# stella-cv/stella_vslam

Measured on AMD Instinct MI355X. Metric: frames/s ORB-extract+match @640x480,2k kpts, higher is better.
Workload: dtype u8

## Files before the change

stella_vslam_amd/csrc/match_kernels.hip:

```cpp
#include "svgpu_internal.h"
#include <algorithm>
#include <cstdlib>
#include "match_kernels.h"
#include "sv_sort.h"
#include "match_device.h"

namespace {
using namespace svmd;

__global__ void k_hamming_pairs(const uint32_t* __restrict__ a, const uint32_t* __restrict__ b, int n, uint32_t* __restrict__ out) {
    const int i = blockIdx.x * blockDim.x + threadIdx.x;
    if (i >= n) return;
    uint32_t q[8];
#pragma unroll
    for (int k = 0; k < 8; ++k) q[k] = a[(size_t)i * 8 + k];
    out[i] = hamming256(q, b + (size_t)i * 8);
}

__global__ __launch_bounds__(256) void k_hamming_matrix(const uint32_t* __restrict__ d1, int n1, const uint32_t* __restrict__ d2,
                                                        int n2, uint16_t* __restrict__ out) {
    __shared__ uint32_t s_t[256 * 8];
    const int j = blockIdx.x * 256 + threadIdx.x;
    uint32_t q[8] = {0, 0, 0, 0, 0, 0, 0, 0};
    if (j < n2)
// ... 251 lines not shown
    uint32_t wq[4][MF_WQ];
#ifdef SV_MF_PAD
    uint32_t pad[SV_MF_PAD];
#endif
};
__device__ __forceinline__ uint32_t mf_row16_max(uint32_t v) {
    v = max(v, (uint32_t)__builtin_amdgcn_update_dpp(0, (int)v, 0x128, 0xF, 0xF, false));
    v = max(v, (uint32_t)__builtin_amdgcn_update_dpp(0, (int)v, 0x124, 0xF, 0xF, false));
    v = max(v, (uint32_t)__builtin_amdgcn_update_dpp(0, (int)v, 0x122, 0xF, 0xF, false));
    v = max(v, (uint32_t)__builtin_amdgcn_update_dpp(0, (int)v, 0x121, 0xF, 0xF, false));
    return v;
}
__device__ __forceinline__ void mf_drain(MfShared& S, const uint32_t* __restrict__ D2, int q_first, int n2c, int wave, int lane, int n, bool ori) {
    for (int e0 = 0; e0 < n; e0 += 64) {
        const int e = e0 + lane;
        bool live = e < n;
        uint32_t key = 0;
        int ql = 0, slot = 0;
        if (live) {
            const uint32_t ent = S.wq[wave][e];
            const int row = (int)(ent >> 16), col = (int)(ent & 0xFFFFu);
            ql = row + wave * MF_QW;
            const uint32_t* q = D2 + (size_t)min(q_first + row, n2c - 1) * 8;
            const uint4 q0 = *reinterpret_cast<const uint4*>(q), q1 = *reinterpret_cast<const uint4*>(q + 4);
            const uint32_t dist = __popc(q0.x ^ S.raw[0][col]) + __popc(q0.y ^ S.raw[1][col]) + __popc(q0.z ^ S.raw[2][col]) + __popc(q0.w ^ S.raw[3][col])
                                  + __popc(q1.x ^ S.raw[4][col]) + __popc(q1.y ^ S.raw[5][col]) + __popc(q1.z ^ S.raw[6][col]) + __popc(q1.w ^ S.raw[7][col]);
            key = (dist << 16) | (uint32_t)S.ridx[col];
            live = S.live[ql] != 0;
            if (ori) live = live && !(fabsf(angle_diff(S.rang[col], S.qa[ql])) > 30.0f);
            if (live) slot = atomicAdd(&S.cnt[ql], 1);
            if (live && slot < MF_SLOTS) S.list[ql][slot] = key;
        }
        unsigned long long ov = __ballot(live && slot >= MF_SLOTS && key < S.rowmax[ql]);
        while (ov) {
            const int src = __ffsll((long long)ov) - 1;
            ov &= ov - 1;
            const uint32_t k = (uint32_t)__builtin_amdgcn_readlane((int)key, src);
            const int row = __builtin_amdgcn_readlane(ql, src);
            uint32_t* R = S.list[row];
            if (k >= S.rowmax[row]) continue;
            const uint32_t v = lane < MF_SLOTS ? R[lane] : 0u;
            const uint32_t vmax = (uint32_t)__builtin_amdgcn_readfirstlane((int)mf_row16_max(v));
            const int arg = __ffsll((long long)__ballot(lane < MF_SLOTS && v == vmax)) - 1;
            uint32_t w = lane == arg ? min(k, vmax) : v;
            if (k < vmax && lane == 0) R[arg] = k;
            w = mf_row16_max(w);
            if (lane == 0) S.rowmax[row] = w;
        }
    }
}
__global__ __launch_bounds__(256, 3) void k_bf_mfma(BfProblem P) {
    __shared__ __attribute__((aligned(16))) MfShared S;
    const int pair = blockIdx.y;
    const int n1 = P.n1_dev ? P.n1_dev[bf_row1(P, pair) * P.n_stride] : P.n1;
    const int n2 = P.n2_dev ? P.n2_dev[pair * P.n_stride] : P.n2;
    const int n1c = min(n1, P.cap1), n2c = min(n2, P.cap2);
    const int tid = threadIdx.x, lane = tid & 63, wave = tid >> 6;
    const int qb = blockIdx.x * MF_QB, q0 = qb + wave * MF_QW;
    if (qb >= n2c) return;
    const uint32_t* __restrict__ D1 = P.sd1 + (size_t)bf_srow1(P, pair) * P.cap1 * 8;
    const float* __restrict__ A1 = P.sa1 + (size_t)bf_srow1(P, pair) * P.cap1;
    const int* __restrict__ I1 = P.si1 + (size_t)bf_srow1(P, pair) * P.cap1;
    const uint32_t* __restrict__ D2 = P.sd2 + (size_t)pair * P.cap2 * 8;
    const float* __restrict__ A2 = P.sa2 + (size_t)pair * P.cap2;
    const int* __restrict__ I2 = P.si2 + (size_t)pair * P.cap2;
    const int* __restrict__ BS1 = P.bs1 + (size_t)bf_srow1(P, pair) * (BF_BINS + 2);
    const bool ori = P.check_orientation != 0;
    const bool prune = ori && bf_prune1(P, pair) && P.prune_ok[pair * 2 + 1];
    S.cnt[tid] = 0;
    S.rowmax[tid] = 0xFFFFFFFFu;
    int my_j = 0;
    {
        const int q = qb + tid;
        bool live = q < n2c;
        if (live) {
            my_j = I2[q];
            live = !P.valid2 || P.valid2[(size_t)pair * P.cap2 + my_j];
        }
        S.qa[tid] = q < n2c ? A2[q] : 0.f;
        S.live[tid] = live ? 1 : 0;
    }
    const int h = lane >> 5;
    v4i A[2][9];
#pragma unroll
    for (int a = 0; a < 2; ++a) {
        const int q = min(q0 + 32 * a + (lane & 31), n2c - 1);
        int pq = 0;
#pragma unroll
        for (int s = 0; s < 8; ++s) {
            const uint32_t w = D2[(size_t)q * 8 + s];
            pq += __popc(w);
            const uint32_t half = (w >> (16 * h)) & 0xFFFFu;
            A[a][s] = v4i{(int)mf_expand02(half & 15u), (int)mf_expand02((half >> 4) & 15u), (int)mf_expand02((half >> 8) & 15u), (int)mf_expand02(half >> 12)};
        }
        const uint2 pp = mf_pop_pieces(pq, true, min((int)P.dmax, 254));
        A[a][8] = h == 0 ? v4i{(int)pp.x, (int)pp.y, 0, 0} : v4i{0, 0, 0, 0};
    }
    int blo[2], bhi[2], wlo[2], whi[2];
    mf_window(A2, BS1, qb, min(qb + MF_QB, n2c) - 1, n1c, prune, blo, bhi);
    const bool wave_live = q0 < n2c;
    mf_window(A2, BS1, min(q0, n2c - 1), min(q0 + MF_QW, n2c) - 1, n1c, prune, wlo, whi);
    const int lt = tid & 31, lw = tid >> 5;
    auto expand = [&](int buf, int tile, int valid) {
        uint4 lo = {0, 0, 0, 0}, hi = {0, 0, 0, 0};
        if (lt < valid) {
            const uint32_t w = S.raw[lw][tile * MF_TT + lt];
            lo.x = mf_expand01(w & 15u);
            lo.y = mf_expand01((w >> 4) & 15u);
            lo.z = mf_expand01((w >> 8) & 15u);
            lo.w = mf_expand01((w >> 12) & 15u);
            hi.x = mf_expand01((w >> 16) & 15u);
            hi.y = mf_expand01((w >> 20) & 15u);
            hi.z = mf_expand01((w >> 24) & 15u);
            hi.w = mf_expand01(w >> 28);
        }
        uint4* B = reinterpret_cast<uint4*>(S.b[buf]) + lw * 64;
        B[lt] = lo;
        B[32 + lt] = hi;
        if (lw == 0) {
            const uint2 pp = lt < valid ? mf_pop_pieces(S.rpop[tile * MF_TT + lt], false, 0) : make_uint2(0x81010101u, 0x01018181u);
            uint4* B8 = reinterpret_cast<uint4*>(S.b[buf]) + 8 * 64;
            B8[lt] = make_uint4(pp.x, pp.y, 0, 0);
            B8[32 + lt] = make_uint4(0, 0, 0, 0);
        }
    };
    int wq_n = 0;
    unsigned n_mine = 0;
    for (int sg = 0; sg < 2; ++sg) {
        const int lo = blo[sg], hi = bhi[sg];
        for (int cbase = lo; cbase < hi; cbase += MF_CH) {
            const int cn = min(MF_CH, hi - cbase), ntiles = (cn + MF_TT - 1) / MF_TT;
            __syncthreads();
            if (tid < cn) {
                const uint4 d0 = *reinterpret_cast<const uint4*>(D1 + (size_t)(cbase + tid) * 8);
                const uint4 d1 = *reinterpret_cast<const uint4*>(D1 + (size_t)(cbase + tid) * 8 + 4);
                S.rang[tid] = A1[cbase + tid];
                S.ridx[tid] = I1[cbase + tid];
                S.rpop[tid] = __popc(d0.x) + __popc(d0.y) + __popc(d0.z) + __popc(d0.w) + __popc(d1.x) + __popc(d1.y) + __popc(d1.z) + __popc(d1.w);
                S.raw[0][tid] = d0.x;
                S.raw[1][tid] = d0.y;
                S.raw[2][tid] = d0.z;
                S.raw[3][tid] = d0.w;
                S.raw[4][tid] = d1.x;
                S.raw[5][tid] = d1.y;
                S.raw[6][tid] = d1.z;
                S.raw[7][tid] = d1.w;
            }
            __syncthreads();
            expand(0, 0, min(MF_TT, cn));
            __syncthreads();
            for (int t = 0, buf = 0; t < ntiles; ++t, buf ^= 1) {
                const int base = cbase + t * MF_TT, tend = min(base + MF_TT, hi);
                const bool mine = wave_live && ((base < whi[0] && tend > wlo[0]) || (base < whi[1] && tend > wlo[1]));
                if (mine) {
                    const v4i* Bf = reinterpret_cast<const v4i*>(S.b[buf]) + lane;
                    v16i acc0 = {}, acc1 = {};
                    v4i b = Bf[0];
#pragma unroll
                    for (int s = 0; s < 9; ++s) {
                        const v4i bn = Bf[(s < 8 ? s + 1 : 0) * 64];
                        acc0 = __builtin_amdgcn_mfma_i32_32x32x32_i8(A[0][s], b, acc0, 0, 0, 0);
                        acc1 = __builtin_amdgcn_mfma_i32_32x32x32_i8(A[1][s], b, acc1, 0, 0, 0);
                        b = bn;
                    }
                    ++n_mine;
                    if (t + 1 < ntiles) expand(buf ^ 1, t + 1, min(MF_TT, cn - (t + 1) * MF_TT));
                    uint32_t m = 0;
#pragma unroll
                    for (int r = 15; r >= 0; --r) m = __builtin_amdgcn_alignbit(m, (uint32_t)acc1[r], 31);
#pragma unroll
                    for (int r = 15; r >= 0; --r) m = __builtin_amdgcn_alignbit(m, (uint32_t)acc0[r], 31);
                    m = ~m;
                    unsigned long long any = __ballot(m != 0);
                    while (any) {
                        int wq = __builtin_amdgcn_readfirstlane(wq_n);
                        if (wq > MF_WQ - 64) {
                            mf_drain(S, D2, q0, n2c, wave, lane, wq, ori);
                            wq = 0;
                        }
                        if (m) {
                            const uint32_t bit = (uint32_t)__ffs((int)m) - 1u;
                            m &= m - 1u;
                            const uint32_t row = ((bit >> 4) << 5) + (bit & 3u) + ((bit & 12u) << 1) + 4u * (uint32_t)h;
                            const int pq = (int)__builtin_amdgcn_mbcnt_hi((uint32_t)(any >> 32), __builtin_amdgcn_mbcnt_lo((uint32_t)any, 0u));
                            S.wq[wave][wq + pq] = (row << 16) | (uint32_t)(t * MF_TT + (lane & 31));
                        }
                        wq_n = wq + __popcll(any);
                        any = __ballot(m != 0);
                    }
                }
                else if (t + 1 < ntiles) expand(buf ^ 1, t + 1, min(MF_TT, cn - (t + 1) * MF_TT));
                __syncthreads();
            }
            mf_drain(S, D2, q0, n2c, wave, lane, __builtin_amdgcn_readfirstlane(wq_n), ori);
            wq_n = 0;
        }
    }
    if (P.mfma_tiles && lane == 0 && n_mine) atomicAdd(P.mfma_tiles, (unsigned long long)n_mine);
    __syncthreads();
    if (qb + tid < n2c) {
        const int cnt = S.cnt[tid], c = min(cnt, MF_SLOTS);
        uint32_t v[MF_SLOTS];
        const uint4* R = reinterpret_cast<const uint4*>(S.list[tid]);
#pragma unroll
        for (int i = 0; i < MF_SLOTS / 4; ++i) {
            const uint4 x = R[i];
            v[4 * i] = x.x;
            v[4 * i + 1] = x.y;
            v[4 * i + 2] = x.z;
            v[4 * i + 3] = x.w;
        }
#pragma unroll
        for (int i = 0; i < MF_SLOTS; ++i) v[i] = i < c ? v[i] : 0xFFFFFFFFu;
#pragma unroll
        for (int k = 2; k <= MF_SLOTS; k <<= 1)
#pragma unroll
            for (int j = k >> 1; j > 0; j >>= 1)
#pragma unroll
                for (int i = 0; i < MF_SLOTS; ++i) {
                    const int l = i ^ j;
                    if (l > i) {
                        const uint32_t lo = min(v[i], v[l]), hi = max(v[i], v[l]);
                        const bool up = (i & k) == 0;
                        v[i] = up ? lo : hi;
                        v[l] = up ? hi : lo;
                    }
                }
        uint4* G = reinterpret_cast<uint4*>(P.topk + ((size_t)pair * P.cap2 + my_j) * BF_LIST);
#pragma unroll
        for (int i = 0; i < MF_SLOTS / 4; ++i) G[i] = make_uint4(v[4 * i], v[4 * i + 1], v[4 * i + 2], v[4 * i + 3]);
        P.cnt[(size_t)pair * P.cap2 + my_j] = cnt;
    }
}

__device__ int bf_decide(const BfProblem& P, int pair, int j, int n1c, const uint4 head, const uint32_t* tail, int cnt, const int* owner) {
    if (cnt == 0) return -1;
    const int m = min(cnt, P.list_k);
    const bool truncated = cnt > P.list_k;
    auto key_at = [&](int k) -> uint32_t { return k == 0 ? head.x : k == 1 ? head.y : k == 2 ? head.z : k == 3 ? head.w : tail[k - 4]; };
    uint32_t a0 = 0xFFFFFFFFu, a1 = 0xFFFFFFFFu;
    for (int k = 0; k < m; ++k) {
        const uint32_t key = key_at(k);
        if (owner[key & 0xFFFFu] < j) continue;
        if (a0 == 0xFFFFFFFFu) a0 = key;
        else {
            a1 = key;
            break;
        }
    }
    const unsigned d_beyond = truncated ? (key_at(m - 1) >> 16) : P.dmax + 1;
    if (a0 != 0xFFFFFFFFu) {
        const unsigned best = a0 >> 16;
        if (HAMMING_DIST_THR_LOW < best) return -1;
        if (a1 != 0xFFFFFFFFu) return (P.lowe_ratio * (float)(a1 >> 16) < (float)best) ? -1 : (int)(a0 & 0xFFFFu);
        if (P.exhaustive && !truncated) return (P.lowe_ratio * (float)MAX_HAMMING_DIST < (float)best) ? -1 : (int)(a0 & 0xFFFFu);
        if (P.lowe_ratio >= 0.f && !(P.lowe_ratio * (float)d_beyond < (float)best)) return (int)(a0 & 0xFFFFu);
    }
    else {
        if (d_beyond > HAMMING_DIST_THR_LOW) return -1;
    }
    return -3;
}

__device__ int bf_full_row(const BfProblem& P, int pair, int j, int n1c, const int* owner, uint32_t* s_best, uint32_t* s_second) {
    const uint32_t* D1 = P.desc1 + (size_t)bf_row1(P, pair) * P.cap1 * 8;
    const uint32_t* D2 = P.desc2 + ((size_t)pair * P.cap2 + j) * 8;
    uint32_t q[8];
#pragma unroll
    for (int k = 0; k < 8; ++k) q[k] = D2[k];
    const float qa = P.angle2[((size_t)pair * P.cap2 + j) * P.angle_stride];
    if (threadIdx.x == 0) {
        *s_best = 0xFFFFFFFFu;
        *s_second = MAX_HAMMING_DIST;
    }
    __syncthreads();
    uint32_t k1 = 0xFFFFFFFFu;
    unsigned d2 = MAX_HAMMING_DIST;
    for (int i = threadIdx.x; i < n1c; i += blockDim.x) {
        if (owner[i] < j) continue;
        if (P.check_orientation && fabsf(angle_diff(P.angle1[((size_t)bf_row1(P, pair) * P.cap1 + i) * P.angle_stride], qa)) > 30.0f) continue;
        const uint32_t key = (hamming256(q, D1 + (size_t)i * 8) << 16) | (uint32_t)i;
        if (key < k1) {
            d2 = min(d2, k1 >> 16);
            k1 = key;
        }
        else d2 = min(d2, key >> 16);
    }
    if (k1 != 0xFFFFFFFFu) atomicMin(s_best, k1);
    __syncthreads();
    const uint32_t kb = *s_best;
    const unsigned mine = (k1 == kb) ? d2 : min(d2, k1 == 0xFFFFFFFFu ? MAX_HAMMING_DIST : (k1 >> 16));
    if (mine < MAX_HAMMING_DIST) atomicMin(s_second, mine);
    __syncthreads();
    const unsigned second = *s_second;
    __syncthreads();
    if (kb == 0xFFFFFFFFu) return -1;
    const unsigned best = kb >> 16;
    if (HAMMING_DIST_THR_LOW < best) return -1;
    if (P.lowe_ratio * (float)second < (float)best) return -1;
    return (int)(kb & 0xFFFFu);
}

template <int BF_RC, int NT>
__global__ __launch_bounds__(NT) void k_bf_replay(BfProblem P, int* __restrict__ g_owner, int* __restrict__ g_match, int use_lds, int pool_rows) {
    extern __shared__ int s_mem[];
    __shared__ int s_changed, s_nund, s_any_und, s_pool_n;
    __shared__ int s_und[1024];
    __shared__ uint32_t s_best, s_second;
    const int pair = blockIdx.x, tid = threadIdx.x, nthr = blockDim.x;
    const int n1 = P.n1_dev ? P.n1_dev[bf_row1(P, pair) * P.n_stride] : P.n1;
    const int n2 = P.n2_dev ? P.n2_dev[pair * P.n_stride] : P.n2;
    const int n1c = min(n1, P.cap1), n2c = min(n2, P.cap2);
    int* owner = use_lds ? s_mem : g_owner + (size_t)pair * P.cap1;
    int* match = use_lds ? s_mem + P.cap1 : g_match + (size_t)pair * P.cap2;
    uint32_t* pool = reinterpret_cast<uint32_t*>(s_mem + (use_lds ? ((P.cap1 + P.cap2 + 3) & ~3) : 0));
    const uint32_t* T = P.topk + (size_t)pair * P.cap2 * BF_LIST;
    const int* C = P.cnt + (size_t)pair * P.cap2;
    for (int i = tid; i < n1c; i += nthr) owner[i] = 0x7FFFFFFF;
    for (int j = tid; j < n2c; j += nthr) match[j] = -2;
    uint4 head[BF_RC];
    int hcnt[BF_RC];
    const uint32_t* tail[BF_RC];
    if (tid == 0) s_pool_n = 0;
    __syncthreads();
#pragma unroll
    for (int u = 0; u < BF_RC; ++u) {
        const int j = u * nthr + tid;
        hcnt[u] = 0;
        head[u] = make_uint4(0xFFFFFFFFu, 0xFFFFFFFFu, 0xFFFFFFFFu, 0xFFFFFFFFu);
        tail[u] = nullptr;
        if (j < n2c) {
            const uint32_t* R = T + (size_t)j * BF_LIST;
            hcnt[u] = C[j];
            head[u] = *reinterpret_cast<const uint4*>(R);
            tail[u] = R + 4;
        }
    }
#pragma unroll
    for (int u = 0; u < BF_RC; ++u)
        if (hcnt[u] > 4 && pool_rows > 0) {
            const int slot = atomicAdd(&s_pool_n, 1);
            if (slot < pool_rows) {
                const uint32_t* R4 = tail[u];
                uint32_t* D = pool + (size_t)slot * (BF_LIST - 4);
#pragma unroll
                for (int i = 0; i < (BF_LIST - 4) / 4; ++i) reinterpret_cast<uint4*>(D)[i] = reinterpret_cast<const uint4*>(R4)[i];
                tail[u] = D;
            }
        }
    __syncthreads();
    for (int sweep = 0; sweep <= n2c; ++sweep) {
        if (tid == 0) {
            s_changed = 0;
            s_any_und = 0;
            s_nund = 0;
        }
        __syncthreads();
        int dec[BF_RC];
        bool und = false;
#pragma unroll
        for (int u = 0; u < BF_RC; ++u) {
            const int j = u * nthr + tid;
            dec[u] = -1;
            if (j < n2c) {
                dec[u] = bf_decide(P, pair, j, n1c, head[u], tail[u], hcnt[u], owner);
                und = und || dec[u] == -3;
            }
        }
        if (und) s_any_und = 1;
        bool changed = false;
        for (int j = BF_RC * nthr + tid; j < n2c; j += nthr) {
            int d = bf_decide(P, pair, j, n1c, *reinterpret_cast<const uint4*>(T + (size_t)j * BF_LIST), T + (size_t)j * BF_LIST + 4, C[j], owner);
            if (d == -3) {
                s_any_und = 1;
                match[j] = -(match[j] + 10);
            }
            else {
                changed = changed || d != match[j];
                match[j] = d;
            }
        }
        __syncthreads();
        if (s_any_und) {
            for (int j0 = 0; j0 < n2c; j0 += nthr) {
                const int j = j0 + tid, u = j0 / nthr;
                bool need = false;
                if (j < n2c) {
                    if (u < BF_RC) {
                        int du = dec[0];
#pragma unroll
                        for (int v = 1; v < BF_RC; ++v)
                            if (v == u) du = dec[v];
                        need = du == -3;
                    }
                    else need = match[j] <= -8;
                }
                if (need) s_und[atomicAdd(&s_nund, 1)] = j;
                __syncthreads();
                const int nund = s_nund;
                int mine = -3;
                for (int k = 0; k < nund; ++k) {
                    const int ju = s_und[k];
                    const int du = bf_full_row(P, pair, ju, n1c, owner, &s_best, &s_second);
                    if (ju == j) mine = du;
                }
                __syncthreads();
                if (tid == 0) s_nund = 0;
                if (need) {
                    if (u < BF_RC) {
#pragma unroll
                        for (int v = 0; v < BF_RC; ++v)
                            if (v == u) dec[v] = mine;
                    }
                    else {
                        changed = changed || mine != -match[j] - 10;
                        match[j] = mine;
                    }
                }
                __syncthreads();
            }
        }
#pragma unroll
        for (int u = 0; u < BF_RC; ++u) {
            const int j = u * nthr + tid;
            if (j < n2c) {
                changed = changed || dec[u] != match[j];
                match[j] = dec[u];
            }
        }
        if (changed) s_changed = 1;
        __syncthreads();
        if (!s_changed) break;
        for (int i = tid; i < n1c; i += nthr) owner[i] = 0x7FFFFFFF;
        __syncthreads();
        for (int j = tid; j < n2c; j += nthr)
            if (match[j] >= 0) atomicMin(&owner[match[j]], j);
        __syncthreads();
    }
    int32_t* out = P.matched + (size_t)pair * P.cap1;
    for (int i = tid; i < P.cap1; i += nthr) out[i] = -1;
    __syncthreads();
    int local = 0;
    for (int j = tid; j < n2c; j += nthr)
        if (match[j] >= 0) {
            out[match[j]] = j;
            ++local;
        }
    if (tid == 0) s_changed = 0;
    __syncthreads();
    if (local) atomicAdd(&s_changed, local);
    __syncthreads();
    if (tid == 0) P.num[pair] = s_changed;
}

#define CAND_SORT_MAX 1024
__device__ __forceinline__ int cand_total(const CandProblem& P) { return P.cand_total ? *P.cand_total : P.cand_off[P.nq]; }
__device__ __forceinline__ bool cand_sorted(const CandProblem& P, int n) { return n <= CAND_SORT_MAX && P.mode != SVGPU_MATCH_TRIANGULATION && P.mode != SVGPU_MATCH_AREA; }
__global__ void k_cand_dist(CandProblem P) {
    if (P.cap > 0 && cand_total(P) > P.cap) return;
    const int q = blockIdx.x;
    if (P.q_valid && !P.q_valid[q]) return;
    const int lo = P.cand_off[q], hi = P.cand_off[q + 1];
    __shared__ unsigned long long s_key[CAND_SORT_MAX];
    const bool long_sorted = hi - lo > 64 && cand_sorted(P, hi - lo);
    uint32_t qd[8];
#pragma unroll
    for (int k = 0; k < 8; ++k) qd[k] = P.qdesc[(size_t)q * 8 + k];
    for (int c = lo + threadIdx.x; c < hi; c += blockDim.x) {
        const int t = P.cand_idx[c];
        bool gated = (P.cand_skip && P.cand_skip[c]) || (P.occupied && P.occupied[t]);
        if (!gated && P.t_xright && 0.f < P.t_xright[t]) {
            const float err = fabsf(P.q_xright[q] - P.t_xright[t]);
            if (P.q_xr_tol[q] < err) gated = true;
        }
        if (!gated && P.check_orientation && fabsf(angle_diff(P.q_angle[q], P.t_angle[t])) > 30.0f) gated = true;
        if (!gated && P.chi_gate) {
            const double e_x = P.q_reproj[2 * q] - (double)P.t_xy[2 * t], e_y = P.q_reproj[2 * q + 1] - (double)P.t_xy[2 * t + 1];
            const double inv_sigma_sq = (double)P.inv_level_sigma_sq[(unsigned)P.t_octave[t]];
            if (P.chi_t_xright && P.chi_t_xright[t] >= 0.f) {
                const float e_xr = P.q_reproj_xr[q] - P.chi_t_xright[t];
                const double err = (e_x * e_x + e_y * e_y) + (double)(e_xr * e_xr);
                if ((double)7.81473f < err * inv_sigma_sq) gated = true;
            }
            else {
                const double err = e_x * e_x + e_y * e_y;
                if ((double)5.99146f < err * inv_sigma_sq) gated = true;
            }
        }
        uint32_t e = 0xFFFFFFFFu;
        if (!gated) {
            const unsigned d = hamming256(qd, P.tdesc + (size_t)t * 8);
            bool useless = false;
            if (P.mode == SVGPU_MATCH_BEST_ONLY) useless = P.thr < d;
            else if (P.mode == SVGPU_MATCH_RATIO_SAME_OCTAVE) useless = !(P.lowe_ratio * (float)d < (float)P.thr) && P.thr < d;
            e = useless ? 0xFFFFFFFFu : ((uint32_t)d << 22) | (uint32_t)t;
        }
        P.dist[c] = e;
        if (long_sorted) s_key[c - lo] = e == 0xFFFFFFFFu ? ~0ull : ((unsigned long long)(e >> 22) << 32) | ((unsigned long long)(c - lo) << 22) | (e & 0x3FFFFFu);
    }
    const int n = hi - lo;
    if (!cand_sorted(P, n)) return;
    if (n <= 64) {
        const int c = lo + (int)threadIdx.x;
        const uint32_t e = c < hi ? P.dist[c] : 0xFFFFFFFFu;
        unsigned long long key = e == 0xFFFFFFFFu ? ~0ull : ((unsigned long long)(e >> 22) << 32) | ((unsigned long long)threadIdx.x << 22) | (e & 0x3FFFFFu);
        const int lane = threadIdx.x;
#pragma unroll
        for (int k = 2; k <= 64; k <<= 1)
#pragma unroll
            for (int j = k >> 1; j > 0; j >>= 1) {
                const unsigned long long other = __shfl_xor(key, j, 64);
                const bool up = (lane & k) == 0, low = (lane & j) == 0;
                const bool take_min = up == low;
                key = take_min ? (key < other ? key : other) : (key < other ? other : key);
            }
        if (c < hi) P.dist[c] = key == ~0ull ? 0xFFFFFFFFu : ((uint32_t)(key >> 32) << 22) | (uint32_t)(key & 0x3FFFFFu);
        return;
    }
    int npow2 = 128;
    while (npow2 < n) npow2 <<= 1;
    for (int i = n + threadIdx.x; i < npow2; i += 64) s_key[i] = ~0ull;
    __syncthreads();
    for (int k = 2; k <= npow2; k <<= 1)
        for (int j = k >> 1; j > 0; j >>= 1) {
            for (int i = threadIdx.x; i < npow2; i += 64) {
                const int p = i ^ j;
                if (p > i) {
                    const unsigned long long a = s_key[i], b = s_key[p];
                    if ((a > b) == ((i & k) == 0)) {
                        s_key[i] = b;
                        s_key[p] = a;
                    }
                }
            }
            __syncthreads();
        }
    for (int i = threadIdx.x; i < n; i += 64) {
        const unsigned long long key = s_key[i];
        P.dist[lo + i] = key == ~0ull ? 0xFFFFFFFFu : ((uint32_t)(key >> 32) << 22) | (uint32_t)(key & 0x3FFFFFu);
    }
}

__device__ __forceinline__ int cand_verdict(const CandProblem& P, unsigned best, unsigned second, int best_lvl, int second_lvl, int best_idx);
__device__ int cand_decide(const CandProblem& P, int q, const int* owner) {
    if (P.q_valid && !P.q_valid[q]) return -1;
    const int lo = P.cand_off[q], hi = P.cand_cnt ? lo + P.cand_cnt[q] : P.cand_off[q + 1];
    if (lo == hi) return -1;
    const bool tri = P.mode == SVGPU_MATCH_TRIANGULATION;
    unsigned best = tri ? P.thr : MAX_HAMMING_DIST, second = MAX_HAMMING_DIST;
    int best_lvl = -1, second_lvl = -1, best_idx = -1;
    if (cand_sorted(P, hi - lo)) {
        for (int c = lo; c < hi; ++c) {
            const uint32_t e = P.dist[c];
            if (e == 0xFFFFFFFFu) break;
            const unsigned d = e >> 22;
            if (d >= MAX_HAMMING_DIST) break;
            const int t = (int)(e & 0x3FFFFFu);
            if (owner[t] < q) continue;
            if (best_idx < 0) {
                best = d;
                best_idx = t;
                best_lvl = P.t_octave ? P.t_octave[t] : 0;
                if (P.mode == SVGPU_MATCH_BEST_ONLY) break;
            }
            else {
                second = d;
                second_lvl = P.t_octave ? P.t_octave[t] : 0;
                break;
            }
        }
    }
    else {
    auto visit = [&](uint32_t e) {
        if (e == 0xFFFFFFFFu) return;
        const unsigned d = e >> 22;
        const int t = (int)(e & 0x3FFFFFu);
        if (owner[t] < q) return;
        if (tri && (P.thr < d || best < d)) return;
        if (d < best) {
            second = best;
            best = d;
            second_lvl = best_lvl;
            best_lvl = P.t_octave ? P.t_octave[t] : 0;
            best_idx = t;
        }
        else if (d < second) {
            second_lvl = P.t_octave ? P.t_octave[t] : 0;
            second = d;
        }
    };
    for (int c = lo; c < hi; c += 4) {
        const uint32_t e0 = P.dist[c], e1 = c + 1 < hi ? P.dist[c + 1] : 0xFFFFFFFFu, e2 = c + 2 < hi ? P.dist[c + 2] : 0xFFFFFFFFu,
                       e3 = c + 3 < hi ? P.dist[c + 3] : 0xFFFFFFFFu;
        visit(e0);
        visit(e1);
        visit(e2);
        visit(e3);
    }
    }
    return cand_verdict(P, best, second, best_lvl, second_lvl, best_idx);
}

__device__ __forceinline__ int cand_verdict(const CandProblem& P, unsigned best, unsigned second, int best_lvl, int second_lvl, int best_idx) {
    if (P.mode == SVGPU_MATCH_RATIO_SAME_OCTAVE) {
        if (best <= P.thr) {
            if (best_lvl == second_lvl && (float)best > P.lowe_ratio * (float)second) return -1;
            return best_idx;
        }
        return -1;
    }
    if (P.mode == SVGPU_MATCH_BEST_ONLY) {
        if (P.thr < best) return -1;
        return best_idx;
    }
    if (P.thr < best || best_idx < 0) return -1;
    if (P.lowe_ratio * (float)second < (float)best) return -1;
    return best_idx;
}

#define SV_LDS __attribute__((address_space(3)))
struct CandLds {
    SV_LDS int* owner;
    SV_LDS int* match;
    SV_LDS int* off;
    SV_LDS int* cnt;
    SV_LDS uint32_t* head;
    SV_LDS uint8_t* occ;
    SV_LDS uint8_t* lvl;
    SV_LDS uint8_t* qv;
    int K;
};
__device__ __forceinline__ int cand_decide_lds(const CandProblem& P, int q, const CandLds& S) {
    const int lo = S.off[q], n = S.cnt ? S.cnt[q] : S.off[q + 1] - lo;
    if (n == 0 || (S.qv && !S.qv[q])) return -1;
    if (!cand_sorted(P, n)) return cand_decide(P, q, (const int*)S.owner);
    unsigned best = MAX_HAMMING_DIST, second = MAX_HAMMING_DIST;
    int best_lvl = -1, second_lvl = -1, best_idx = -1;
    bool done = false;
    auto take_loaded = [&](uint32_t e, int own, int lv) {
        if (done) return;
        if (e == 0xFFFFFFFFu || (e >> 22) >= MAX_HAMMING_DIST) {
            done = true;
            return;
        }
        const int t = (int)(e & 0x3FFFFFu);
        if (own < q) return;
        if (best_idx < 0) {
            best = e >> 22;
            best_idx = t;
            best_lvl = lv;
            if (P.mode == SVGPU_MATCH_BEST_ONLY) done = true;
        }
        else {
            second = e >> 22;
            second_lvl = lv;
            done = true;
        }
    };
    auto take = [&](uint32_t e) {
        if (done || e == 0xFFFFFFFFu) {
            take_loaded(e, 0, 0);
            return;
        }
        const int t = (int)(e & 0x3FFFFFu);
        take_loaded(e, S.owner[t], S.lvl ? (int)S.lvl[t] : 0);
    };
    const int nk = min(n, S.K);
    const SV_LDS uint32_t* h = S.head + (size_t)q * S.K;
    for (int k0 = 0; k0 < nk && !done; k0 += 4) {
        uint32_t e[4];
        int own[4], lv[4];
#pragma unroll
        for (int j = 0; j < 4; ++j) e[j] = k0 + j < nk ? h[k0 + j] : 0xFFFFFFFFu;
#pragma unroll
        for (int j = 0; j < 4; ++j) {
            const int t = e[j] == 0xFFFFFFFFu ? 0 : (int)(e[j] & 0x3FFFFFu);
            own[j] = S.owner[t];
            lv[j] = S.lvl ? (int)S.lvl[t] : 0;
        }
        const bool best_only = P.mode == SVGPU_MATCH_BEST_ONLY;
#pragma unroll
        for (int j = 0; j < 4; ++j) {
            const unsigned d = e[j] >> 22;
            const bool padding = k0 + j >= nk;
            const bool stop = !padding && (e[j] == 0xFFFFFFFFu || d >= MAX_HAMMING_DIST), active = !done;
            const bool avail = active && !padding && !stop && own[j] >= q, first = avail && best_idx < 0, sec = avail && best_idx >= 0;
            best = first ? d : best;
            best_lvl = first ? lv[j] : best_lvl;
            second = sec ? d : second;
            second_lvl = sec ? lv[j] : second_lvl;
            best_idx = first ? (int)(e[j] & 0x3FFFFFu) : best_idx;
            done = done || (active && stop) || sec || (first && best_only);
        }
    }
    for (int c = lo + nk; c < lo + n && !done; c += 4) {
        const int hi = lo + n;
        const uint32_t e0 = P.dist[c], e1 = c + 1 < hi ? P.dist[c + 1] : 0xFFFFFFFFu, e2 = c + 2 < hi ? P.dist[c + 2] : 0xFFFFFFFFu,
                       e3 = c + 3 < hi ? P.dist[c + 3] : 0xFFFFFFFFu;
        take(e0);
        take(e1);
        take(e2);
        take(e3);
    }
    return cand_verdict(P, best, second, best_lvl, second_lvl, best_idx);
}
#define CAND_LDS_BUDGET (150 * 1024)
__host__ __device__ inline size_t cand_lds_bytes(int nq, int nt, int K, bool with_cnt = false) {
    return (size_t)(nt + nq + nq + 1 + (with_cnt ? nq : 0)) * 4 + (size_t)nq * K * 4 + 2 * (((size_t)nt + 3) & ~size_t(3)) + (((size_t)nq + 3) & ~size_t(3)) + 16;
}
#define CAND_CHUNK_QPT 1
__global__ __launch_bounds__(1024) void k_cand_replay_lds(CandProblem P, int K) {
    extern __shared__ int s_cand[];
    __shared__ int s_changed;
    if (P.cap > 0 && cand_total(P) > P.cap) {
        if (P.num_host && threadIdx.x == 0) P.num_host[0] = 0, P.num_host[1] = cand_total(P);
        return;
    }
    const int tid = threadIdx.x, nthr = blockDim.x;
    const int nt = P.nt_dev ? min(*P.nt_dev, P.nt) : P.nt;
    CandLds S;
    S.owner = (SV_LDS int*)s_cand;
    S.match = S.owner + P.nt;
    S.off = S.match + P.nq;
    S.cnt = P.cand_cnt ? S.off + P.nq + 1 : nullptr;
    S.head = (SV_LDS uint32_t*)(S.off + P.nq + 1 + (P.cand_cnt ? P.nq : 0));
    SV_LDS uint8_t* bytes = (SV_LDS uint8_t*)(S.head + (size_t)P.nq * K);
    S.occ = P.occupied ? bytes : nullptr;
    S.lvl = P.t_octave ? bytes + ((P.nt + 3) & ~3) : nullptr;
    S.qv = P.q_valid ? bytes + 2 * ((P.nt + 3) & ~3) : nullptr;
    S.K = K;
    for (int q = tid; q <= P.nq; q += nthr) {
        S.off[q] = P.cand_off[q];
        if (S.cnt && q < P.nq) S.cnt[q] = P.cand_cnt[q];
        if (S.qv && q < P.nq) S.qv[q] = P.q_valid[q];
    }
    for (int t = tid; t < nt; t += nthr) {
        S.owner[t] = (P.occupied && P.occupied[t]) ? -1 : 0x7FFFFFFF;
        if (S.lvl) S.lvl[t] = (uint8_t)P.t_octave[t];
    }
    S.occ = nullptr;
    __syncthreads();
    for (int i = tid; i < P.nq * K; i += nthr) {
        const int q = i / K, k = i - q * K, lo = S.off[q], n = S.cnt ? S.cnt[q] : S.off[q + 1] - lo;
        if (k < n) S.head[i] = P.dist[lo + k];
    }
    if (tid == 0) s_changed = 0;
    __syncthreads();
    if (P.dbg_phase == 1) return;
    int local = 0, sweeps_total = 0;
    const int chunk = nthr * CAND_CHUNK_QPT;
    for (int lo = 0; lo < P.nq; lo += chunk) {
        int mine[CAND_CHUNK_QPT], prev[CAND_CHUNK_QPT];
#pragma unroll
        for (int u = 0; u < CAND_CHUNK_QPT; ++u) mine[u] = -2, prev[u] = -1;
        for (int sweep = 0; sweep <= chunk; ++sweep) {
// ... 259 lines not shown
        const int t = P.cand_idx[lo + (int)(kb & 0xFFFFFu)];
        if (lane == 0) {
            const int prev = (int)ld(reinterpret_cast<unsigned*>(&holder[t]));
            if (0 <= prev) st(reinterpret_cast<unsigned*>(&match[prev]), 0xFFFFFFFFu);
            st(reinterpret_cast<unsigned*>(&match[q]), (unsigned)t);
            st(reinterpret_cast<unsigned*>(&holder[t]), (unsigned)q);
            st(&mdist[t], best);
        }
        __syncthreads();
    }
    int local = 0;
    __syncthreads();
    for (int q = lane; q < P.nq; q += 64) {
        const int m = (int)ld(reinterpret_cast<const unsigned*>(&match[q]));
        P.match_q[q] = m;
        local += m >= 0;
    }
#pragma unroll
    for (int off = 32; off > 0; off >>= 1) local += __shfl_xor(local, off, 64);
    if (lane == 0) *P.num = local;
}

__device__ __forceinline__ int wave_sum_i(int v) {
#pragma unroll
    for (int off = 32; off > 0; off >>= 1) v += __shfl_xor(v, off, 64);
    return v;
}
struct StereoPair {
    const svgpu_keypoint *kl, *kr;
    const uint32_t *dl, *dr;
    int nl, nr;
    float *xr, *depth, *corr;
    int32_t *row_off, *row_fill, *row_items;
};
__device__ __forceinline__ StereoPair stereo_pair(const StereoProblem& P, int pair) {
    StereoPair Q;
    const size_t o = P.nl_dev ? (size_t)pair * P.cap : 0;
    Q.nl = P.nl_dev ? min(P.nl_dev[(size_t)pair * P.n_stride], P.cap) : P.nl;
    Q.nr = P.nr_dev ? min(P.nr_dev[(size_t)pair * P.n_stride], P.cap) : P.nr;
    Q.kl = P.kl + o, Q.kr = P.kr + o, Q.dl = P.dl + o * 8, Q.dr = P.dr + o * 8;
    Q.xr = P.xr + o, Q.depth = P.depth + o, Q.corr = P.corr + o;
    const int nr_cap = P.nl_dev ? P.cap : P.nr;
    Q.row_off = P.row_off + (size_t)pair * (P.rows + 1);
    Q.row_fill = P.row_fill + (size_t)pair * P.rows;
    Q.row_items = P.row_items + (size_t)pair * nr_cap * P.rows_per_kp;
    return Q;
}
__device__ __forceinline__ void stereo_band(const StereoProblem& P, const svgpu_keypoint& r, int& min_r, int& max_r) {
    const float rad = 2.0f * P.sf[r.octave];
    max_r = min((int)ceil((double)(r.y + rad)), P.rows - 1);
    min_r = max((int)floor((double)(r.y - rad)), 0);
}
template <bool FILL>
__global__ __launch_bounds__(256) void k_stereo_rows(StereoProblem P) {
    const StereoPair Q = stereo_pair(P, blockIdx.y);
    const int ir = blockIdx.x * 256 + threadIdx.x;
    if (ir >= Q.nr) return;
    int min_r, max_r;
    stereo_band(P, Q.kr[ir], min_r, max_r);
    for (int row = min_r; row <= max_r; ++row) {
        if (FILL) Q.row_items[Q.row_off[row] + atomicAdd(&Q.row_fill[row], 1)] = ir;
        else atomicAdd(&Q.row_off[row], 1);
    }
}
__global__ __launch_bounds__(1024) void k_stereo_rows_scan(StereoProblem P) {
    __shared__ int s_part[1024];
    __shared__ int s_carry;
    int32_t* off = P.row_off + (size_t)blockIdx.x * (P.rows + 1);
    const int tid = threadIdx.x, n = P.rows;
    if (tid == 0) s_carry = 0;
    __syncthreads();
    for (int base = 0; base < n; base += 1024) {
        const int i = base + tid;
        const int v = i < n ? off[i] : 0;
        int incl = v;
#pragma unroll
        for (int d = 1; d < 64; d <<= 1) {
            const int t = __shfl_up(incl, d, 64);
            if ((tid & 63) >= d) incl += t;
        }
        if ((tid & 63) == 63) s_part[tid >> 6] = incl;
        __syncthreads();
        int before = 0;
        for (int w = 0; w < (tid >> 6); ++w) before += s_part[w];
        const int carry = s_carry;
        if (i < n) off[i] = carry + before + incl - v;
        __syncthreads();
        if (tid == 1023) s_carry = carry + before + incl;
        __syncthreads();
    }
    if (tid == 0) off[n] = s_carry;
}
__global__ __launch_bounds__(256) void k_stereo(StereoProblem P) {
    const int il = blockIdx.x * 4 + __builtin_amdgcn_readfirstlane(threadIdx.x >> 6), lane = threadIdx.x & 63;
    const int pair = blockIdx.y;
    const StereoPair Q = stereo_pair(P, pair);
    if (il >= Q.nl) return;
    const svgpu_keypoint k = Q.kl[il];
    const int lvl = k.octave;
    float out_xr = -1.0f, out_depth = -1.0f, out_corr = -1.0f;
    const int row = (int)k.y;
    const float min_x_right = k.x - P.max_disp, max_x_right = k.x - P.min_disp;
    uint32_t best = 0xFFFFFFFFu;
    if (!(max_x_right < 0) && row >= 0 && row < P.rows) {
        uint32_t q[8];
#pragma unroll
        for (int w = 0; w < 8; ++w) q[w] = Q.dl[(size_t)il * 8 + w];
        for (int c = Q.row_off[row] + lane; c < Q.row_off[row + 1]; c += 64) {
            const int ir = Q.row_items[c];
            const svgpu_keypoint r = Q.kr[ir];
            if (r.octave < lvl - 1 || r.octave > lvl + 1) continue;
            if (r.x < min_x_right || max_x_right < r.x) continue;
            const unsigned d = hamming256(q, Q.dr + (size_t)ir * 8);
            if (d < P.thr) best = min(best, (d << 16) | (uint32_t)ir);
        }
    }
#pragma unroll
    for (int off = 32; off > 0; off >>= 1) best = min(best, (uint32_t)__shfl_xor((int)best, off, 64));
    if (best != 0xFFFFFFFFu) {
        const float x_right = Q.kr[best & 0xFFFFu].x;
        const float isf = P.isf[lvl];
        const int sxl = __float2int_rn(k.x * isf), syl = __float2int_rn(k.y * isf), sxr = __float2int_rn(x_right * isf);
        const int ini_x = sxr - 10, end_x = sxr + 10;
        const bool ok = !(ini_x < 0 || P.w[lvl] <= end_x) && syl - 5 >= 0 && syl + 5 < P.h[lvl] && sxl - 5 >= 0 && sxl + 5 < P.w[lvl];
        if (ok) {
            const uint8_t* PL = P.lev_l[lvl] + (size_t)pair * (lvl == 0 ? P.img_stride_l : P.pyr_stride_l);
            const uint8_t* PR = P.lev_r[lvl] + (size_t)pair * (lvl == 0 ? P.img_stride_r : P.pyr_stride_r);
            const int pl = P.pitch_l[lvl], pr = P.pitch_r[lvl];
            const int lc = PL[__umul24(syl, pl) + sxl];
            int a[2], dy[2], dx[2];
            bool has[2];
#pragma unroll
            for (int t = 0; t < 2; ++t) {
                const int p = lane + 64 * t;
                has[t] = p < 121;
                dy[t] = has[t] ? p / 11 - 5 : 0;
                dx[t] = has[t] ? p % 11 - 5 : 0;
                a[t] = has[t] ? (int)PL[__umul24(syl + dy[t], pl) + sxl + dx[t]] - lc : 0;
            }
            float corr[11];
            float best_corr = 3.402823466e+38f;
            int best_off = 0;
#pragma unroll
            for (int o = 0; o < 11; ++o) {
                const int off = o - 5;
                const int rc = PR[__umul24(syl, pr) + sxr + off];
                int acc = 0;
#pragma unroll
                for (int t = 0; t < 2; ++t)
                    if (has[t]) {
                        const int b = (int)PR[__umul24(syl + dy[t], pr) + sxr + off + dx[t]] - rc;
                        acc += abs(a[t] - b);
                    }
                const float c = (float)wave_sum_i(acc);
                corr[o] = c;
                if (c < best_corr) {
                    best_corr = c;
                    best_off = off;
                }
            }
            if (best_off != -5 && best_off != 5) {
                float c1 = corr[0], c2 = corr[1], c3 = corr[2];
#pragma unroll
                for (int o = 1; o < 10; ++o)
                    if (o == best_off + 5) {
                        c1 = corr[o - 1];
                        c2 = corr[o];
                        c3 = corr[o + 1];
                    }
                const float x_delta = (float)((double)(c1 - c3) / (2.0 * (double)(c1 + c3) - 4.0 * (double)c2));
                if (!((double)x_delta < -1.0 || 1.0 < (double)x_delta)) {
                    float best_x_right = P.sf[lvl] * ((float)(sxr + best_off) + x_delta);
                    float best_disp = k.x - best_x_right;
                    if (!(best_disp < P.min_disp || P.max_disp <= best_disp)) {
                        if (best_disp <= 0.0f) {
                            best_disp = 0.01f;
                            best_x_right = k.x - best_disp;
                        }
                        out_depth = P.fxb / best_disp;
                        out_xr = best_x_right;
                        out_corr = best_corr;
                    }
                }
            }
        }
    }
    if (lane == 0) {
        Q.xr[il] = out_xr;
        Q.depth[il] = out_depth;
        Q.corr[il] = out_corr;
    }
}

#define STEREO_MEDIAN_LDS 32768
__global__ __launch_bounds__(1024) void k_stereo_median(StereoProblem P) {
    __shared__ int s_cnt[16];
    __shared__ unsigned short s_c[STEREO_MEDIAN_LDS];
    const int pair = blockIdx.x, tid = threadIdx.x, nthr = blockDim.x;
    const int nl = P.nl_dev ? min(P.nl_dev[(size_t)pair * P.n_stride], P.cap) : P.nl;
    const size_t o = P.nl_dev ? (size_t)pair * P.cap : 0;
    float* xr = P.xr + o;
    float* depth = P.depth + o;
    const float* corr = P.corr + o;
    const bool staged = nl <= STEREO_MEDIAN_LDS;
    if (staged)
        for (int i = tid; i < nl; i += nthr) s_c[i] = (xr[i] != -1.0f || depth[i] != -1.0f) ? (unsigned short)(int)corr[i] : (unsigned short)0xFFFF;
    __syncthreads();
    auto count_le = [&](int v) -> int {
        int c = 0;
        if (staged) {
            for (int i = tid; i < nl; i += nthr) {
                const int x = s_c[i];
                c += (x != 0xFFFF && (v < 0 || x <= v)) ? 1 : 0;
            }
        }
        else {
            for (int i = tid; i < nl; i += nthr)
                if (xr[i] != -1.0f || depth[i] != -1.0f) c += (v < 0 || (int)corr[i] <= v) ? 1 : 0;
        }
        for (int off = 32; off > 0; off >>= 1) c += __shfl_xor(c, off, 64);
        __syncthreads();
        if ((tid & 63) == 0) s_cnt[tid >> 6] = c;
        __syncthreads();
        int t = 0;
        for (int w = 0; w < (nthr >> 6); ++w) t += s_cnt[w];
        return t;
    };
    const int kept = count_le(-1);
    if (kept == 0) return;
    const int rank = kept / 2;
    int lo = 0, hi = 1 << 17;
    while (lo < hi) {
        const int mid = (lo + hi) >> 1;
        if (count_le(mid) > rank) hi = mid;
        else lo = mid + 1;
    }
    const float thr = (float)(2.0 * (double)(float)lo);
    for (int i = tid; i < nl; i += nthr)
        if ((xr[i] != -1.0f || depth[i] != -1.0f) && thr < (float)(int)corr[i]) {
            xr[i] = -1.0f;
            depth[i] = -1.0f;
        }
}

}

void sv_launch_stereo(svgpu_ctx* ctx, hipStream_t s, const StereoProblem& P, int pairs) {
    SvProfScope ps(ctx, s, "k_stereo");
    const int nl = P.nl_dev ? P.cap : P.nl, nr = P.nl_dev ? P.cap : P.nr;
    if (nl <= 0 || pairs <= 0) return;
    (void)hipMemsetAsync(P.row_off, 0, (size_t)pairs * (P.rows + 1) * 4, s);
    (void)hipMemsetAsync(P.row_fill, 0, (size_t)pairs * P.rows * 4, s);
    if (nr > 0) hipLaunchKernelGGL(k_stereo_rows<false>, dim3((nr + 255) / 256, pairs), dim3(256), 0, s, P);
    hipLaunchKernelGGL(k_stereo_rows_scan, dim3(pairs), dim3(1024), 0, s, P);
    if (nr > 0) hipLaunchKernelGGL(k_stereo_rows<true>, dim3((nr + 255) / 256, pairs), dim3(256), 0, s, P);
    hipLaunchKernelGGL(k_stereo, dim3((nl + 3) / 4, pairs), dim3(256), 0, s, P);
}
void sv_launch_stereo_median(hipStream_t s, const StereoProblem& P, int pairs) {
    if (pairs > 0) hipLaunchKernelGGL(k_stereo_median, dim3(pairs), dim3(1024), 0, s, P);
}

void sv_launch_hamming_pairs(hipStream_t s, const uint32_t* a, const uint32_t* b, int n, uint32_t* out) {
    if (n <= 0) return;
    hipLaunchKernelGGL(k_hamming_pairs, dim3((n + 255) / 256), dim3(256), 0, s, a, b, n, out);
}
void sv_launch_hamming_matrix(hipStream_t s, const uint32_t* d1, int n1, const uint32_t* d2, int n2, uint16_t* out) {
    if (n1 <= 0 || n2 <= 0) return;
    hipLaunchKernelGGL(k_hamming_matrix, dim3((n2 + 255) / 256), dim3(256), 0, s, d1, n1, d2, n2, out);
}
void sv_launch_bf(svgpu_ctx* ctx, hipStream_t s, const BfProblem& P0, int pairs, int* g_owner, int* g_match) {
    if (pairs <= 0) return;
    BfProblem P = P0;
    if (P.lowe_ratio > 0.f && 50.0f / P.lowe_ratio + 2.0f < 256.0f) P.dmax = (unsigned)(50.0f / P.lowe_ratio) + 2u;
    else P.dmax = 256u;
    if (P.dmax < 50u) P.dmax = 50u;
    P.exhaustive = P.dmax >= 256u;
    static const bool force_valu = getenv("SVGPU_BF_VALU") != nullptr;
    {
        SvProfScope ps(ctx, s, "k_bf_binsort");
        P.shared_sort = P.ring1 == pairs && P.desc1 == P.desc2 && P.angle1 == P.angle2 && P.n1_dev == P.n2_dev && P.cap1 == P.cap2;
        if (P.shared_sort) {
            P.sd1 = P.sd2;
            P.sa1 = P.sa2;
            P.si1 = P.si2;
            P.bs1 = P.bs2;
        }
        hipLaunchKernelGGL(k_bf_binsort, dim3(pairs, P.shared_sort ? 1 : 2), dim3(256), 0, s, P);
    }
    {
        SvProfScope ps(ctx, s, "k_bf_topk");
        if (P.dmax >= 128u || force_valu) {
            P.list_k = BF_K;
            hipLaunchKernelGGL(k_bf_topk, dim3((P.cap2 + BF_QB - 1) / BF_QB, pairs), dim3(256), 0, s, P);
        }
        else {
            P.list_k = MF_SLOTS;
            P.mfma_tiles = sv_prof_counter(ctx, "k_bf_topk");
            hipLaunchKernelGGL(k_bf_mfma, dim3((P.cap2 + MF_QB - 1) / MF_QB, pairs), dim3(256), 0, s, P);
        }
    }
    SvProfScope ps(ctx, s, "k_bf_replay");
    size_t lds = (size_t)((P.cap1 + P.cap2 + 3) & ~3) * sizeof(int);
    const int use_lds = lds <= 96 * 1024;
    if (!use_lds) lds = 0;
    const int pool_rows = (int)std::min<size_t>(1024, (128 * 1024 - lds) / ((BF_LIST - 4) * sizeof(uint32_t)));
    lds += (size_t)pool_rows * (BF_LIST - 4) * sizeof(uint32_t);
    if (P.cap2 <= 5 * 512) {
        (void)sv_allow_dynamic_lds(reinterpret_cast<const void*>(k_bf_replay<5, 512>), 144 * 1024);
        hipLaunchKernelGGL((k_bf_replay<5, 512>), dim3(pairs), dim3(512), lds, s, P, g_owner, g_match, use_lds, pool_rows);
    }
    else {
        (void)sv_allow_dynamic_lds(reinterpret_cast<const void*>(k_bf_replay<4, 1024>), 144 * 1024);
        hipLaunchKernelGGL((k_bf_replay<4, 1024>), dim3(pairs), dim3(1024), lds, s, P, g_owner, g_match, use_lds, pool_rows);
    }
}
static void grid_scan(hipStream_t s, int32_t* data, int n) {
    if (n <= 16384) sv_scan_i32(s, data, n, nullptr);
    else hipLaunchKernelGGL(k_exclusive_scan, dim3(1), dim3(1024), 0, s, data, n);
}
void sv_launch_grid_frame(hipStream_t s, const GridProblem& G) {
    const int nc = G.cols * G.rows;
    if (nc <= GRID_ONE_CELLS && G.nt <= 1024 * GRID_ONE_KPT_ROUNDS && !std::getenv("SVGPU_GRID_FOUR_LAUNCHES")) {
        hipLaunchKernelGGL(k_grid_frame_one, dim3(1), dim3(1024), 0, s, G);
        return;
    }
    (void)hipMemsetAsync(G.cell_off, 0, (size_t)(nc + 1) * sizeof(int32_t), s);
    if (G.nt > 0) hipLaunchKernelGGL(k_grid_assign, dim3((G.nt + 255) / 256), dim3(256), 0, s, G);
    grid_scan(s, G.cell_off, nc);
    if (G.nt > 0) hipLaunchKernelGGL(k_grid_place, dim3((G.nt + 255) / 256), dim3(256), 0, s, G);
}
void sv_launch_grid_queries(hipStream_t s, const GridProblem& G) {
    if (G.nq > 0) hipLaunchKernelGGL(k_grid_walk<false>, dim3((G.nq + 3) / 4), dim3(256), 0, s, G);
    grid_scan(s, G.cand_off, G.nq);
}
void sv_launch_grid_build(hipStream_t s, const GridProblem& G) {
    sv_launch_grid_frame(s, G);
    sv_launch_grid_queries(s, G);
}
void sv_launch_grid_fill(hipStream_t s, const GridProblem& G) {
    if (G.nq > 0) hipLaunchKernelGGL(k_grid_walk<true>, dim3((G.nq + 3) / 4), dim3(256), 0, s, G);
}
int sv_cand_replay_form(int nq, int nt, bool with_cnt, int mode) {
    if (mode == SVGPU_MATCH_AREA) return (size_t)(2 * (size_t)nt + (size_t)nq) * sizeof(int) <= 60 * 1024 ? 1 : 0;
    const size_t tables = cand_lds_bytes(nq, nt, 0, with_cnt);
    if (tables > CAND_LDS_BUDGET) return -1;
    return nq > 0 ? (int)std::min<size_t>(64, (CAND_LDS_BUDGET - tables) / ((size_t)nq * 4)) : 0;
}
void sv_launch_cand(svgpu_ctx* ctx, hipStream_t s, const CandProblem& P, int* owner, int* match, unsigned* mdist) {
    SvProfScope ps(ctx, s, "k_cand");
    if (P.nq > 0) hipLaunchKernelGGL(k_cand_dist, dim3(P.nq), dim3(64), 0, s, P);
    if (P.mode == SVGPU_MATCH_AREA) {
        const size_t lds = (size_t)(2 * P.nt + P.nq) * sizeof(int);
        const int use_lds = sv_cand_replay_form(P.nq, P.nt, false, P.mode);
        hipLaunchKernelGGL(k_area_replay, dim3(1), dim3(64), use_lds ? lds : 0, s, P, owner, match, mdist, use_lds);
        return;
    }
    sv_launch_cand_replay(ctx, s, P, owner, match);
}
void sv_launch_cand_replay(svgpu_ctx* ctx, hipStream_t s, const CandProblem& P0, int* owner, int* match) {
    CandProblem P = P0;
    static const int dbg = std::getenv("SVGPU_REPLAY_DBG") ? std::atoi(std::getenv("SVGPU_REPLAY_DBG")) : 0;
    P.dbg_phase = dbg;
    const bool wc = P.cand_cnt != nullptr;
    const int K = sv_cand_replay_form(P.nq, P.nt, wc, P.mode);
    if (K >= 0) {
        (void)sv_allow_dynamic_lds((const void*)k_cand_replay_lds, CAND_LDS_BUDGET);
        hipLaunchKernelGGL(k_cand_replay_lds, dim3(1), dim3(1024), cand_lds_bytes(P.nq, P.nt, K, wc), s, P, K);
    }
    else hipLaunchKernelGGL(k_cand_replay, dim3(1), dim3(1024), 0, s, P, owner, match);
}
```

Baseline: 283,800.

## Add register-resident incremental BF match replay kernel for small problems

Adds a new k_bf_replay kernel that keeps per-row match state in registers, with only the owner array in LDS. Each sweep re-decides only rows above the lowest changed index and stops once nothing changes. Ownership is reclaimed incrementally rather than rebuilt every pass, and the output count uses wave ballots. The old kernel becomes k_bf_replay_full and is kept as the fallback for large problems, while the new kernel is used when the arrays fit in LDS and cap2 is at most 2560. The goal is fewer LDS accesses and less per-sweep work in the iterative replay, at the cost of more complex convergence logic and a fixed pool of 512 rows.

```diff
diff --git a/stella_vslam_amd/csrc/match_kernels.hip b/stella_vslam_amd/csrc/match_kernels.hip
--- a/stella_vslam_amd/csrc/match_kernels.hip
+++ b/stella_vslam_amd/csrc/match_kernels.hip
@@ -577,7 +577,7 @@
 }
 
 template <int BF_RC, int NT>
-__global__ __launch_bounds__(NT) void k_bf_replay(BfProblem P, int* __restrict__ g_owner, int* __restrict__ g_match, int use_lds, int pool_rows) {
+__global__ __launch_bounds__(NT) void k_bf_replay_full(BfProblem P, int* __restrict__ g_owner, int* __restrict__ g_match, int use_lds, int pool_rows) {
     extern __shared__ int s_mem[];
     __shared__ int s_changed, s_nund, s_any_und, s_pool_n;
     __shared__ int s_und[1024];
@@ -726,6 +726,150 @@
     if (local) atomicAdd(&s_changed, local);
     __syncthreads();
     if (tid == 0) P.num[pair] = s_changed;
+}
+
+#define BF_POOL_ROWS 512
+#ifndef BF_REPLAY_WAVES
+#define BF_REPLAY_WAVES 8
+#endif
+template <int BF_RC, int NT>
+__global__ __launch_bounds__(NT, BF_REPLAY_WAVES) void k_bf_replay(BfProblem P, int pool_rows) {
+    extern __shared__ int s_mem[];
+    __shared__ int s_minchg[2], s_flag[2], s_nund, s_pool_n, s_count;
+    __shared__ int s_und[NT];
+    __shared__ uint32_t s_best, s_second;
+    constexpr int NONE = 0x7FFFFFFF;
+    const int pair = blockIdx.x, tid = threadIdx.x;
+    const int n1 = P.n1_dev ? P.n1_dev[bf_row1(P, pair) * P.n_stride] : P.n1;
+    const int n2 = P.n2_dev ? P.n2_dev[pair * P.n_stride] : P.n2;
+    const int n1c = min(n1, P.cap1), n2c = min(n2, P.cap2);
+    int* owner = s_mem;
+    uint32_t* pool = reinterpret_cast<uint32_t*>(s_mem + ((P.cap1 + 3) & ~3));
+    const uint32_t* T = P.topk + (size_t)pair * P.cap2 * BF_LIST;
+    const int* C = P.cnt + (size_t)pair * P.cap2;
+    for (int i = tid; i < n1c; i += NT) owner[i] = NONE;
+    if (tid == 0) {
+        s_pool_n = s_count = s_nund = 0;
+        s_minchg[0] = s_minchg[1] = NONE;
+        s_flag[0] = s_flag[1] = 0;
+    }
+    __syncthreads();
+    uint4 head[BF_RC];
+    int hcnt[BF_RC], cur[BF_RC];
+    int slot[BF_RC];
+    unsigned live = 0;
+    auto tail_of = [&](int u, int j) -> const uint32_t* { return slot[u] >= 0 ? pool + slot[u] * (BF_LIST - 4) : T + (size_t)j * BF_LIST + 4; };
+#pragma unroll
+    for (int u = 0; u < BF_RC; ++u) {
+        const int j = u * NT + tid;
+        hcnt[u] = 0;
+        cur[u] = -1;
+        head[u] = make_uint4(0xFFFFFFFFu, 0xFFFFFFFFu, 0xFFFFFFFFu, 0xFFFFFFFFu);
+        slot[u] = -1;
+        if (j < n2c) {
+            hcnt[u] = C[j];
+            head[u] = *reinterpret_cast<const uint4*>(T + (size_t)j * BF_LIST);
+        }
+    }
+#pragma unroll
+    for (int u = 0; u < BF_RC; ++u) {
+        if (hcnt[u] > 0 && (head[u].x >> 16) <= HAMMING_DIST_THR_LOW) live |= 1u << u;
+        if (hcnt[u] > 4 && ((live >> u) & 1u)) {
+            const int sl = atomicAdd(&s_pool_n, 1);
+            if (sl < pool_rows) {
+                const uint32_t* R4 = T + (size_t)(u * NT + tid) * BF_LIST + 4;
+                uint32_t* D = pool + sl * (BF_LIST - 4);
+#pragma unroll
+                for (int i = 0; i < (BF_LIST - 4) / 4; ++i) reinterpret_cast<uint4*>(D)[i] = reinterpret_cast<const uint4*>(R4)[i];
+                slot[u] = sl;
+            }
+        }
+    }
+    __syncthreads();
+    int m_prev = -1;
+    for (int sweep = 0; sweep <= n2c; ++sweep) {
+        const int par = sweep & 1;
+        int dec[BF_RC], lowest = NONE;
+        bool und = false;
+#pragma unroll
+        for (int u = BF_RC - 1; u >= 0; --u) {
+            const int j = u * NT + tid;
+            dec[u] = cur[u];
+            if ((live >> u) & 1u) {
+                if (j <= m_prev) live &= ~(1u << u);
+                else {
+                    dec[u] = bf_decide(P, pair, j, n1c, head[u], tail_of(u, j), hcnt[u], owner);
+                    if (dec[u] == -3) und = true;
+                    else if (dec[u] != cur[u]) lowest = j;
+                }
+            }
+        }
+        if (und) atomicOr(&s_flag[par], 2);
+        if (lowest != NONE) atomicMin(&s_minchg[par], lowest);
+        __syncthreads();
+        if (s_flag[par] & 2) {
+#pragma unroll
+            for (int u = 0; u < BF_RC; ++u) {
+                if (u * NT >= n2c) break;
+                const int j = u * NT + tid;
+                const bool need = dec[u] == -3;
+                if (need) s_und[atomicAdd(&s_nund, 1)] = j;
+                __syncthreads();
+                const int nund = s_nund;
+                int mine = -3;
+                for (int k = 0; k < nund; ++k) {
+                    const int ju = s_und[k];
+                    const int du = bf_full_row(P, pair, ju, n1c, owner, &s_best, &s_second);
+                    if (ju == j) mine = du;
+                }
+                __syncthreads();
+                if (tid == 0) s_nund = 0;
+                if (need) {
+                    dec[u] = mine;
+                    if (mine != cur[u]) atomicMin(&s_minchg[par], j);
+                }
+                __syncthreads();
+            }
+        }
+        const int m = s_minchg[par];
+        if (tid == 0) {
+            s_minchg[par ^ 1] = NONE;
+            s_flag[par ^ 1] = 0;
+        }
+        if (m == NONE) break;
+        bool reset = false;
+#pragma unroll
+        for (int u = 0; u < BF_RC; ++u) {
+            const int j = u * NT + tid;
+            if (dec[u] != cur[u] && cur[u] >= 0 && owner[cur[u]] == j) {
+                owner[cur[u]] = NONE;
+                reset = true;
+            }
+        }
+        if (reset) atomicOr(&s_flag[par], 1);
+        __syncthreads();
+        const bool reclaim = (s_flag[par] & 1) != 0;
+#pragma unroll
+        for (int u = 0; u < BF_RC; ++u) {
+            const int j = u * NT + tid;
+            const bool changed = dec[u] != cur[u];
+            cur[u] = dec[u];
+            if (cur[u] >= 0 && (changed || reclaim) && owner[cur[u]] > j) atomicMin(&owner[cur[u]], j);
+        }
+        __syncthreads();
+        m_prev = m;
+    }
+    int32_t* out = P.matched + (size_t)pair * P.cap1;
+    int local = 0;
+    for (int i0 = 0; i0 < P.cap1; i0 += NT) {
+        const int i = i0 + tid;
+        const int o = i < n1c ? owner[i] : NONE;
+        if (i < P.cap1) out[i] = o != NONE ? o : -1;
+        local += __popcll(__ballot(o != NONE));
+    }
+    if ((tid & 63) == 0 && local) atomicAdd(&s_count, local);
+    __syncthreads();
+    if (tid == 0) P.num[pair] = s_count;
 }
 
 #define CAND_SORT_MAX 1024
@@ -1591,16 +1735,22 @@
     SvProfScope ps(ctx, s, "k_bf_replay");
     size_t lds = (size_t)((P.cap1 + P.cap2 + 3) & ~3) * sizeof(int);
     const int use_lds = lds <= 96 * 1024;
+    if (use_lds && P.cap2 <= 5 * 512) {
+        lds = (size_t)((P.cap1 + 3) & ~3) * sizeof(int) + (size_t)BF_POOL_ROWS * (BF_LIST - 4) * sizeof(uint32_t);
+        (void)sv_allow_dynamic_lds(reinterpret_cast<const void*>(k_bf_replay<5, 512>), 144 * 1024);
+        hipLaunchKernelGGL((k_bf_replay<5, 512>), dim3(pairs), dim3(512), lds, s, P, BF_POOL_ROWS);
+        return;
+    }
     if (!use_lds) lds = 0;
     const int pool_rows = (int)std::min<size_t>(1024, (128 * 1024 - lds) / ((BF_LIST - 4) * sizeof(uint32_t)));
     lds += (size_t)pool_rows * (BF_LIST - 4) * sizeof(uint32_t);
     if (P.cap2 <= 5 * 512) {
-        (void)sv_allow_dynamic_lds(reinterpret_cast<const void*>(k_bf_replay<5, 512>), 144 * 1024);
-        hipLaunchKernelGGL((k_bf_replay<5, 512>), dim3(pairs), dim3(512), lds, s, P, g_owner, g_match, use_lds, pool_rows);
+        (void)sv_allow_dynamic_lds(reinterpret_cast<const void*>(k_bf_replay_full<5, 512>), 144 * 1024);
+        hipLaunchKernelGGL((k_bf_replay_full<5, 512>), dim3(pairs), dim3(512), lds, s, P, g_owner, g_match, use_lds, pool_rows);
     }
     else {
-        (void)sv_allow_dynamic_lds(reinterpret_cast<const void*>(k_bf_replay<4, 1024>), 144 * 1024);
-        hipLaunchKernelGGL((k_bf_replay<4, 1024>), dim3(pairs), dim3(1024), lds, s, P, g_owner, g_match, use_lds, pool_rows);
+        (void)sv_allow_dynamic_lds(reinterpret_cast<const void*>(k_bf_replay_full<4, 1024>), 144 * 1024);
+        hipLaunchKernelGGL((k_bf_replay_full<4, 1024>), dim3(pairs), dim3(1024), lds, s, P, g_owner, g_match, use_lds, pool_rows);
     }
 }
 static void grid_scan(hipStream_t s, int32_t* data, int n) {
```

New measurement: 285,600, median of 6. About the same (+0.6%).
